# A-Kokolis/Hermes

Hardware: AMD Instinct MI355X
Metric: replicated KVS ops/s (reads+writes committed) (higher is better)
Workload: dtype u8

## Files before the change

### hermes_amd/csrc/hkv_batch.hip

```cpp
#include <hip/hip_runtime.h>

#include <algorithm>
#include <cstdio>
#include <cstdlib>
#include <cstring>

#include "hkv_batch_dev.h"

namespace hkv {

__host__ __device__ constexpr int rounds_for(int type, bool rmw)
{
    return type == kVals || (type == kLocal && !rmw) ? 0 : 2;
}

enum : uint8_t { kIvRaise = 1, kIvEq = 2, kIvWrite = 4, kIvCand = 8, kIvApply = 16 };
constexpr int64_t kInvDirectMax = 1 << 23;

enum : uint8_t { kAkMatch = 1 };

__device__ __forceinline__ uint8_t ack_opcode(uint8_t in) { return in == kLastAckSuccess ? in : kAckSuccess; }

__device__ __forceinline__ uint8_t inv_opcode(uint8_t in, bool oog)
{
// ... 1012 lines not shown
            const unsigned long long v = ((unsigned long long)(~a.rtag0) << 32) | (uint32_t)gi[k];
            const unsigned long long old = atomicExch(a.fw + fw_index(a, phys[k]), v);
            if ((uint32_t)(old >> 32) == ~a.rtag0 && a.error_flags) atomicOr(a.error_flags, 16u);
        }
        uint8_t *entry = a.log + phys[k];
        Ctx c = make_ctx(a);
        uint8_t idx = 0;
        if (TYPE == kAcks) {
            uint8_t *xx;
            elem_at(a, (uint32_t)gi[k], xx, idx, c);
        }
        Meta t = m[k];
        dispatch<SV>(TYPE, x, entry, idx, t, c);
        if (!meta_equal(t, m[k])) meta_store(entry, t);
    }
}

__device__ __forceinline__ uint4 load_chunk(const uint8_t *x, int q, int32_t esz)
{
    if (16 * q + 16 <= esz) return *reinterpret_cast<const uint4 *>(x + 16 * q);
    if (16 * q + 8 <= esz) {
        const uint64_t t = *reinterpret_cast<const uint64_t *>(x + 16 * q);
        return make_uint4((uint32_t)t, (uint32_t)(t >> 32), 0u, 0u);
    }
    return make_uint4(0u, 0u, 0u, 0u);
}

__device__ __forceinline__ bool chunk_equal(const uint4 &a, const uint4 &b)
{
    return a.x == b.x && a.y == b.y && a.z == b.z && a.w == b.w;
}

template <int TYPE, bool IL = false>
__global__ __launch_bounds__(64) void k_unique_lds(BatchArgs a)
{
    constexpr int P = 1;
    constexpr int E = 16 * P;
    __shared__ uint4 sops[E * 4];
    __shared__ uint4 sln[E * 4];
    __shared__ uint32_t sent[E];
    __shared__ uint8_t sprb[E];
    const int tid = threadIdx.x, q = tid & 3, gbase = tid & ~3;
    const int64_t i0 = (int64_t)blockIdx.x * E;
    const int64_t n_live = a.offsets ? (int64_t)a.offsets[a.n_batches] : a.n;
    uint64_t key[P];
    bool probe[P], ok[P], live[P];
    uint64_t phys[P];
    uint4 ln[P], op[P];
    int te[P];
#pragma unroll
    for (int k = 0; k < P; ++k) {
        te[k] = k * 16 + (tid >> 2);
        const int64_t i = i0 + te[k];
        live[k] = i < a.n && i < n_live;
        op[k] = live[k] ? load_chunk(a.elems + i * a.esz, q, a.esz) : make_uint4(0u, 0u, 0u, 0u);
        sops[te[k] * 4 + q] = op[k];
    }
#pragma unroll
    for (int k = 0; k < P; ++k) {
        key[k] = (uint64_t)(uint32_t)__shfl((int)op[k].x, 0, 4) | ((uint64_t)(uint32_t)__shfl((int)op[k].y, 0, 4) << 32);
        const uint32_t h0 = (uint32_t)__shfl((int)op[k].z, 0, 4);
        probe[k] = false;
        const int64_t i = i0 + te[k];
        if (live[k] && (a.offsets || in_count(a, (uint32_t)i))) {
            if (!skip_elem_os(TYPE, (uint8_t)h0, (uint8_t)(h0 >> 8))) {
                probe[k] = true;
            } else if (TYPE == kInvs && a.ns_idx && q == 0) {
                int64_t start;
                const int32_t b = batch_of(a, i, start);
                atomicMax(&a.ns_idx[b], (int32_t)(i - start));
            }
        }
    }
    uint8_t *home[P];
    lookup_pair<P, IL>(a, key, probe, q, gbase, ok, phys, ln, home);
#pragma unroll
    for (int k = 0; k < P; ++k) {
        Meta m;
        const uint64_t ek = line_key_meta(ln[k], m);
        const bool hit = ok[k] && ek == key[k];
        sln[te[k] * 4 + q] = ln[k];
        if (q == 0) {
            sent[te[k]] = hit ? (uint32_t)(phys[k] / a.g.entry_unit) : kNone;
            sprb[te[k]] = probe[k];
        }
    }
    __syncthreads();
    if (tid < E && i0 + tid < n_live) {
        const int64_t i = i0 + tid;
        uint8_t *x = reinterpret_cast<uint8_t *>(&sops[tid * 4]);
        uint8_t *ent = reinterpret_cast<uint8_t *>(&sln[tid * 4]);
        const uint32_t e = sent[tid];
        if (e != kNone) {
            if (a.check_unique) {
                const unsigned long long v = ((unsigned long long)(~a.rtag0) << 32) | (uint32_t)i;
                const unsigned long long old = atomicExch(a.fw + fw_index(a, phys_of(a, e)), v);
                if ((uint32_t)(old >> 32) == ~a.rtag0 && a.error_flags) atomicOr(a.error_flags, 16u);
            }
            Ctx c = make_ctx(a);
            int done = -1;
            if (TYPE == kAcks) c.rw_done = &done;
            Meta m;
            meta_load(ent, m);
            Meta t = m;
            dispatch<31>(TYPE, x, ent, 0, t, c);
            if (!meta_equal(t, m)) meta_store(ent, t);
            if (TYPE == kAcks && done >= 0 && a.rw) {
                uint8_t *xx;
                uint8_t idx;
                elem_at(a, (uint32_t)i, xx, idx, c);
                complete_rw_slot(c, done);
            }
        } else if (sprb[tid]) {
            x[9] = kMiss;
        }
    }
    __syncthreads();
#pragma unroll
    for (int k = 0; k < P; ++k) {
        if (!live[k]) continue;
        uint4 w = sops[te[k] * 4 + q];
        if (TYPE == kInvs && a.ack_out) {
            uint8_t *y = a.ack_out + (i0 + te[k]) * a.ack_out_size;
            const uint32_t hz = sops[te[k] * 4].z;
            const uint8_t oc = (uint8_t)hz;
            const bool full = oc == kOpInvAbort && a.ack_out_size >= (uint32_t)a.esz;
            if (oc == kInvSuccess || full) {
                uint4 c = w;
                if (q == 0)
                    c.z = (hz & ~0xFFFFu) | (oc == kInvSuccess ? kOpAck : kOpInvAbort) |
                          ((uint32_t)(uint8_t)a.g.machine_id << 8);
                if (q == 0 || (full && 16 * q < a.esz)) {
                    if (16 * q + 16 <= a.esz || q == 0) *reinterpret_cast<uint4 *>(y + 16 * q) = c;
                    else *reinterpret_cast<uint64_t *>(y + 16 * q) = (uint64_t)c.x | ((uint64_t)c.y << 32);
                }
            } else if (q == 0) {
                y[8] = kEmpty;
            }
            if (q == 0 && (oc == kInvSuccess || oc == kOpInvAbort || oc == kOpMembChange))
                w.z = (w.z & ~0xFFu) | kEmpty;
        }
        if (!chunk_equal(w, op[k])) {
            uint8_t *xg = a.elems + (i0 + te[k]) * a.esz + 16 * q;
            if (16 * q + 16 <= a.esz) *reinterpret_cast<uint4 *>(xg) = w;
            else *reinterpret_cast<uint64_t *>(xg) = (uint64_t)w.x | ((uint64_t)w.y << 32);
        }
        if (ok[k] && q > 0) {
            const uint4 l = sln[te[k] * 4 + q];
            if (!chunk_equal(l, ln[k])) reinterpret_cast<uint4 *>(IL ? home[k] : a.log + phys[k])[q] = l;
        }
    }
}

template <int TYPE, int RMAX, int CH, bool IL = false>
__global__ __launch_bounds__(64) void k_unique_rows(BatchArgs a)
{
    constexpr int P = kLookupPair;
    constexpr int E = 16 * P;
    __shared__ uint4 sops[RMAX][E * CH];
    __shared__ uint4 sln[E * 4];
    __shared__ uint32_t sent[E];
    __shared__ uint8_t spart[E];
    const int tid = threadIdx.x, q = tid & 3, gbase = tid & ~3;
    const int64_t i0 = (int64_t)blockIdx.x * E;
    const int R = a.n_rows < RMAX ? a.n_rows : RMAX;
    const int64_t n_live = a.offsets ? (int64_t)a.offsets[a.n_batches] : a.n;
    uint64_t key[P];
    bool probe[P], ok[P], live[P];
    uint64_t phys[P];
    uint4 ln[P], op[RMAX][P];
    uint32_t part[P];
    int te[P];
#pragma unroll
    for (int k = 0; k < P; ++k) {
        te[k] = k * 16 + (tid >> 2);
        const int64_t i = i0 + te[k];
        live[k] = i < a.n && i < n_live && (a.offsets || in_count(a, (uint32_t)i));
#pragma unroll
        for (int r = 0; r < RMAX; ++r) {
            const bool on = live[k] && r < R && r != a.skip_row;
            op[r][k] = on && q < CH ? load_chunk(a.elems + (r * a.row_stride + i) * a.esz, q, a.esz)
                                    : make_uint4(0u, 0u, 0u, 0u);
            if (q < CH) sops[r][te[k] * CH + q] = op[r][k];
        }
    }
#pragma unroll
    for (int k = 0; k < P; ++k) {
        uint64_t kk = 0;
        uint32_t p = 0;
        bool mismatch = false;
#pragma unroll
        for (int r = 0; r < RMAX; ++r) {
            const uint64_t kr = (uint64_t)(uint32_t)__shfl((int)op[r][k].x, 0, 4) |
                                ((uint64_t)(uint32_t)__shfl((int)op[r][k].y, 0, 4) << 32);
            const uint32_t h0 = (uint32_t)__shfl((int)op[r][k].z, 0, 4);
            if (!live[k] || r >= R || r == a.skip_row || (uint8_t)h0 == 0) continue;
            if (skip_elem_os(TYPE, (uint8_t)h0, (uint8_t)(h0 >> 8))) continue;
            if (p && kr != kk) mismatch = true;
            if (!p) kk = kr;
            p |= 1u << r;
        }
        if (mismatch && q == 0 && a.error_flags) atomicOr(a.error_flags, 16u);
        key[k] = kk;
        part[k] = mismatch ? 0u : p;
        probe[k] = part[k] != 0;
    }
    uint8_t *home[P];
    lookup_pair<P, IL>(a, key, probe, q, gbase, ok, phys, ln, home);
#pragma unroll
    for (int k = 0; k < P; ++k) {
        Meta m;
        const uint64_t ek = line_key_meta(ln[k], m);
        const bool hit = ok[k] && ek == key[k];
        sln[te[k] * 4 + q] = ln[k];
        if (q == 0) {
            sent[te[k]] = hit ? (uint32_t)(phys[k] / a.g.entry_unit) : kNone;
            spart[te[k]] = (uint8_t)part[k];
        }
    }
    __syncthreads();
    if (tid < E && i0 + tid < n_live) {
        const int64_t i = i0 + tid;
        uint8_t *ent = reinterpret_cast<uint8_t *>(&sln[tid * 4]);
        const uint32_t e = sent[tid];
        const uint32_t p = spart[tid];
        if (e != kNone && p) {
            if (a.check_unique) {
                const unsigned long long v = ((unsigned long long)(~a.rtag0) << 32) | (uint32_t)i;
                const unsigned long long old = atomicExch(a.fw + fw_index(a, phys_of(a, e)), v);
                if ((uint32_t)(old >> 32) == ~a.rtag0 && a.error_flags) atomicOr(a.error_flags, 16u);
            }
            Ctx c = make_ctx(a);
            int done = -1;
            if (TYPE == kAcks) c.rw_done = &done;
            Meta m;
            meta_load(ent, m);
            Meta t = m;
#pragma unroll
            for (int r = 0; r < RMAX; ++r)
                if ((p >> r) & 1u) dispatch<31>(TYPE, reinterpret_cast<uint8_t *>(&sops[r][tid * CH]), ent, 0, t, c);
            if (!meta_equal(t, m)) meta_store(ent, t);
            if (TYPE == kAcks && done >= 0 && a.rw) {
                uint8_t *xx;
                uint8_t idx;
                elem_at(a, (uint32_t)i, xx, idx, c);
                complete_rw_slot(c, done);
            }
        } else {
#pragma unroll
            for (int r = 0; r < RMAX; ++r)
                if ((p >> r) & 1u) reinterpret_cast<uint8_t *>(&sops[r][tid * CH])[9] = kMiss;
        }
    }
    __syncthreads();
#pragma unroll
    for (int k = 0; k < P; ++k) {
        if (!live[k]) continue;
#pragma unroll
        for (int r = 0; r < RMAX; ++r) {
            if (r >= R || r == a.skip_row || q >= CH) continue;
            uint4 w = sops[r][te[k] * CH + q];
            if (TYPE == kAcks && CH == 1 && a.ack_out) {
                const uint8_t oc = (uint8_t)w.z;
                uint4 v = make_uint4(0u, 0u, (uint32_t)kEmpty, 0u);
                if (oc != 0 && oc != kAckSuccess && oc != kOpMembChange && oc != kEmpty)
                    v = make_uint4(w.x, w.y, (w.z & ~0xFFFFu) | (uint32_t)kOpVal | ((uint32_t)(uint8_t)a.g.machine_id << 8), w.w);
                *reinterpret_cast<uint4 *>(a.ack_out + (r * a.row_stride + i0 + te[k]) * 16) = v;
                if (oc != 0 && oc != kEmpty) w.z = (w.z & ~0xFFu) | (uint32_t)kEmpty;
            }
            if (!chunk_equal(w, op[r][k])) {
                uint8_t *xg = a.elems + (r * a.row_stride + i0 + te[k]) * a.esz + 16 * q;
                if (16 * q + 16 <= a.esz) *reinterpret_cast<uint4 *>(xg) = w;
                else *reinterpret_cast<uint64_t *>(xg) = (uint64_t)w.x | ((uint64_t)w.y << 32);
            }
        }
        if (ok[k] && q > 0) {
            const uint4 l = sln[te[k] * 4 + q];
            if (!chunk_equal(l, ln[k])) reinterpret_cast<uint4 *>(IL ? home[k] : a.log + phys[k])[q] = l;
        }
    }
}

constexpr int kUbElems = 16;
constexpr int kUbChunks = 20;
template <int TYPE>
__global__ __launch_bounds__(64) void k_unique_big(BatchArgs a)
{
    __shared__ uint4 sx[kUbElems * kUbChunks];
    __shared__ uint4 se[kUbElems * kUbChunks];
    constexpr int kPerLane = (kUbChunks + 3) / 4;
    uint4 x0[kPerLane], e0[kPerLane];
    const int tid = threadIdx.x, q = tid & 3, el = tid >> 2, gbase = tid & ~3;
    const int64_t i = (int64_t)blockIdx.x * kUbElems + el;
    const bool live = i < a.n;
    const int nch = (a.esz + 15) / 16;
    uint8_t *xg = a.elems + i * a.esz;
#pragma unroll
    for (int u = 0; u < kPerLane; ++u) {
        const int c = q + 4 * u;
        const uint4 v = live && c < nch ? load_chunk(xg, c, a.esz) : make_uint4(0u, 0u, 0u, 0u);
        if (c < nch) sx[el * kUbChunks + c] = v;
        x0[u] = v;
    }
    const uint4 c0 = sx[el * kUbChunks];
    const uint64_t key = (uint64_t)c0.x | ((uint64_t)c0.y << 32);
    bool probe = false;
    if (live && (a.offsets || in_count(a, (uint32_t)i))) {
        if (!skip_elem_os(TYPE, (uint8_t)c0.z, (uint8_t)(c0.z >> 8))) {
            probe = true;
        } else if (TYPE == kInvs && a.ns_idx && q == 0) {
            int64_t start;
            const int32_t b = batch_of(a, i, start);
            atomicMax(&a.ns_idx[b], (int32_t)(i - start));
        }
    }
    bool ok;
    uint64_t phys;
    uint4 ln;
    lookup_pair<1>(a, &key, &probe, q, gbase, &ok, &phys, &ln);
    Meta m0;
    const uint64_t ek = line_key_meta(ln, m0);
    const bool hit = ok && ek == key;
#pragma unroll
    for (int u = 0; u < kPerLane; ++u) e0[u] = make_uint4(0u, 0u, 0u, 0u);
    if (hit) {
        const uint4 *eg = reinterpret_cast<const uint4 *>(a.log + phys);
#pragma unroll
        for (int u = 0; u < kPerLane; ++u) {
            const int c = q + 4 * u;
            if (c >= kUbChunks) continue;
            const uint4 v = c < 4 ? ln : eg[c];
            se[el * kUbChunks + c] = v;
            e0[u] = v;
        }
    }
    __syncthreads();
    if (q == 0 && live) {
        uint8_t *x = reinterpret_cast<uint8_t *>(&sx[el * kUbChunks]);
        uint8_t *ent = reinterpret_cast<uint8_t *>(&se[el * kUbChunks]);
        if (hit) {
            if (a.check_unique) {
                const unsigned long long v = ((unsigned long long)(~a.rtag0) << 32) | (uint32_t)i;
                const unsigned long long old = atomicExch(a.fw + fw_index(a, phys), v);
                if ((uint32_t)(old >> 32) == ~a.rtag0 && a.error_flags) atomicOr(a.error_flags, 16u);
            }
            Ctx c = make_ctx(a);
            int done = -1;
            if (TYPE == kAcks) c.rw_done = &done;
            Meta m;
            meta_load(ent, m);
            Meta t = m;
            dispatch<287>(TYPE, x, ent, 0, t, c);
            if (!meta_equal(t, m)) meta_store(ent, t);
            if (TYPE == kAcks && done >= 0 && a.rw) {
                uint8_t *xx;
                uint8_t idx;
                elem_at(a, (uint32_t)i, xx, idx, c);
                complete_rw_slot(c, done);
            }
        } else if (probe) {
            x[9] = kMiss;
        }
    }
    __syncthreads();
    if (live) {
        const uint32_t hz = sx[el * kUbChunks].z;
        const uint8_t oc = (uint8_t)hz;
        if (TYPE == kInvs && a.ack_out) {
            uint8_t *y = a.ack_out + i * a.ack_out_size;
            const bool full = oc == kOpInvAbort && a.ack_out_size >= (uint32_t)a.esz;
            if (oc == kInvSuccess || full) {
                for (int c = q; c < (full ? nch : 1); c += 4) {
                    uint4 w = sx[el * kUbChunks + c];
                    if (c == 0)
                        w.z = (hz & ~0xFFFFu) | (oc == kInvSuccess ? kOpAck : kOpInvAbort) |
                              ((uint32_t)(uint8_t)a.g.machine_id << 8);
                    if (16 * c + 16 <= a.esz || c == 0) *reinterpret_cast<uint4 *>(y + 16 * c) = w;
                    else *reinterpret_cast<uint64_t *>(y + 16 * c) = (uint64_t)w.x | ((uint64_t)w.y << 32);
                }
            } else if (q == 0) {
                y[8] = kEmpty;
            }
        }
#pragma unroll
        for (int u = 0; u < kPerLane; ++u) {
            const int c = q + 4 * u;
            if (c >= nch) continue;
            uint4 w = sx[el * kUbChunks + c];
            if (TYPE == kInvs && a.ack_out && c == 0 && (oc == kInvSuccess || oc == kOpInvAbort || oc == kOpMembChange))
                w.z = (w.z & ~0xFFu) | kEmpty;
            if (chunk_equal(w, x0[u])) continue;
            if (16 * c + 16 <= a.esz) *reinterpret_cast<uint4 *>(xg + 16 * c) = w;
            else *reinterpret_cast<uint64_t *>(xg + 16 * c) = (uint64_t)w.x | ((uint64_t)w.y << 32);
        }
    }
    if (hit) {
        uint4 *eg = reinterpret_cast<uint4 *>(a.log + phys);
#pragma unroll
        for (int u = 0; u < kPerLane; ++u) {
            const int c = q + 4 * u;
            if (c >= kUbChunks) continue;
            const uint4 w = se[el * kUbChunks + c];
            if (c > 0 && !chunk_equal(w, e0[u])) eg[c] = w;
        }
    }
}

template <int TYPE, int SV>
__global__ __launch_bounds__(256) void k_resolve(BatchArgs a, int r)
{
    extern __shared__ uint64_t sx[];
    const bool kStage = SV == 31 && a.esz <= 16;
    const int64_t i = (int64_t)blockIdx.x * 256 + threadIdx.x;
    bool left = false;
    VCopy vc{nullptr, nullptr};
    VCopy *vcp = SV != 31 && a.g.st_value <= 320 ? &vc : nullptr;
    const bool wave_shadow = SV != 31 && vcp;
    bool cand = false;
    uint32_t prev = 0;
    if (i < a.n && a.st[i] == kStPend) {
        const uint32_t e = a.ent[i];
        const uint32_t f = first_cand(*fw_of(a, e), a.rtag0 + (uint32_t)r);
        prev = a.pf[i];
        if (f == kNone || (uint32_t)i <= f) {
            uint8_t *xg = a.elems + i * a.esz;
            uint8_t *xl = reinterpret_cast<uint8_t *>(sx) + threadIdx.x * (uint32_t)a.esz;
            if (kStage) copy_elem(xl, xg, a.esz);
// ... 748 lines not shown
    BatchLaunch bl{};
    return carve(bl, 0, cap, entry_size);
}

void batch_carve(BatchLaunch &bl, uint8_t *base, int64_t cap, uint32_t entry_size)
{
    carve(bl, reinterpret_cast<uintptr_t>(base), cap, entry_size);
}

size_t batch_fw_words(uint64_t log_cap) { return (size_t)(log_cap >> 6); }

uint32_t batch_max_epoch() { return (1u << 29) - 1; }

static BatchPlan plan_batch(const BatchLaunch &bl)
{
    BatchPlan p{};
    const int64_t n = bl.n;
    if (n <= 0) return p;
    const int32_t type = bl.type;
    const uint32_t sv = bl.g.st_value;
    const bool rmw = bl.g.rmw_enabled != 0;
    const bool geo64 = sv == 31 && bl.g.entry_size == 64;
    const bool local_type = type == kLocal || type == kLocalAfterMemb;
    p.sv = sv == 31 ? 31 : sv == 287 ? 287 : 0;
    p.big = bl.esz > 64;
    p.mixed = bl.hdr != nullptr;
    p.il = bl.line != nullptr;
    p.inv_direct = type == kInvs && !rmw && n < kInvDirectMax;
    p.ack_direct = type == kAcks && !rmw && n < (int64_t)kNone;
    p.ack_out = bl.ack_out && (type == kInvs || (type == kAcks && bl.n_rows > 0));
    p.state_out = local_type;
    p.opc = type == kLocal;
    p.fk = type == kLocal && rmw && p.big;
    p.rw_mirrors = type == kAcks;

    if ((bl.path == kPathSmall || (bl.path == kPathAuto && n <= kSmallMaxElems)) && n <= kSmallMaxElems) {
        p.engine = Engine::kSmall;
    } else if (type == kLocal && !rmw && bl.esz == 56 && geo64 && !bl.offsets) {
        p.engine = Engine::kLocalDirect;
        p.inline_instance = true;
    } else if (bl.n_rows > 0 && bl.unique) {
        p.engine = Engine::kRows;
        p.rmax = bl.n_rows <= 2 ? 2 : 8;
        p.ch = type == kInvs ? 4 : bl.esz <= 16 ? 1 : 4;
        p.inline_instance = geo64 && !local_type && bl.n_rows <= 8;
    } else if (bl.unique && (type == kInvs || type == kAcks)) {
        if (geo64 && bl.esz <= 64) {
            p.engine = Engine::kUniqueLds64;
            p.inline_instance = true;
        } else if (type == kInvs && sv == 287 && bl.g.entry_size == 320 && bl.esz <= 320) {
            p.engine = Engine::kUniqueLdsBig;
        } else {
            p.engine = Engine::kUniqueInPlace;
            if (p.ack_out) p.refuse = -1;
        }
    } else if (type == kVals) {
        p.engine = Engine::kValsOnePass;
        p.inline_instance = geo64;
    } else {
        p.lookup_head = local_type && n > kLookupHead ? kLookupHead : n;
        p.slab_threads = p.big ? 128 : 256;
        p.engine = p.ack_direct ? Engine::kRoundsAckDirect
                   : p.inv_direct ? Engine::kRoundsInvDirect
                   : p.big && type != kInvs ? Engine::kRoundsInPlace
                                            : Engine::kRoundsSlab;
    }
    if (p.il && !p.inline_instance) p.refuse = -1;
    if (bl.region_bytes && p.engine != Engine::kSmall) p.refuse = -1;
    p.node_suspected = p.engine != Engine::kSmall && type == kInvs && bl.ns_idx && bl.node_suspected;

    const uint32_t vend = (uint32_t)kOpValueOff + sv;
    if (!bl.patch) p.patches = Patches::kNone;
    else if (p.engine == Engine::kSmall) p.patches = Patches::kApplyFirst;
    else if (p.engine == Engine::kLocalDirect) p.patches = Patches::kByEngine;
    else if (type == kLocal && p.big && !bl.offsets && sv != 31 && sv <= kPirMaxValue && bl.esz % 8 == 0 &&
             (uint32_t)bl.esz >= vend && (uint32_t)bl.esz <= vend + 8)
        p.patches = Patches::kInResolve;
    else p.patches = Patches::kApplyFirst;
    return p;
}

bool batch_inline_capable(const BatchLaunch &bl) { return plan_batch(bl).inline_instance; }

static BatchArgs make_args(const BatchLaunch &bl, const BatchPlan &p)
{
#ifdef HKV_DEBUG_MODES
    static const int dbg_env = getenv("HKV_DBG") ? atoi(getenv("HKV_DBG")) : 0;
#else
    constexpr int dbg_env = 0;
#endif
    static const int check_unique_env = getenv("HKV_CHECK_UNIQUE") ? atoi(getenv("HKV_CHECK_UNIQUE")) : 0;
    BatchArgs a{};
    a.elems = bl.elems;
    a.counts = bl.counts;
    a.offsets = bl.offsets;
    a.index = bl.index;
    a.log = bl.log;
    a.rw = bl.rw;
    a.ns_idx = bl.ns_idx;
    a.fw = bl.fw;
    a.fx = bl.fx;
    a.fy = bl.fy;
    a.ft = bl.ft;
    a.fw_mask = (uint32_t)((bl.g.log_cap >> 6) - 1);
    a.ent = bl.ent;
    a.st = bl.st;
    a.pf = bl.pf;
    a.shadow = bl.shadow;
    a.mem = bl.mem;
    a.fbl = bl.fbl;
    a.ctr = bl.ctr;
    a.error_flags = bl.error_flags;
    a.g = bl.g;
    a.n = bl.n;
    a.rw_stride = bl.rw_stride;
    a.stride = bl.stride;
    a.esz = bl.esz;
    a.type = bl.type;
    a.rtag0 = bl.epoch << 3;
    a.ltag = (uint8_t)(bl.epoch % 255u + 1u);
    a.rounds = rounds_for(bl.type, bl.g.rmw_enabled != 0);
    a.inv_direct = p.inv_direct;
    a.ack_direct = p.ack_direct;
    a.g_membership = bl.g_membership;
    a.w_ack_init = bl.w_ack_init;
    a.node_suspected = bl.node_suspected;
    a.n_batches = bl.n_batches;
    a.host_src = bl.host_src;
    a.host_dst = bl.host_dst;
    a.dev_region = bl.dev_region;
    a.region_bytes = bl.region_bytes;
    a.done_flag = bl.done_flag;
    a.done_value = bl.done_value;
    a.hdr = bl.hdr;
    a.state_out = p.state_out ? bl.state_out : nullptr;
    a.opc = p.opc ? bl.opcode_in : nullptr;
    a.patch = p.patches == Patches::kInResolve || p.patches == Patches::kByEngine ? bl.patch : nullptr;
    a.fk = p.fk ? bl.fk : nullptr;
    a.hx = p.patches == Patches::kInResolve ? bl.hx : nullptr;
    a.rws = p.rw_mirrors ? bl.rw_state : nullptr;
    a.rwo = p.rw_mirrors ? bl.opcode_in : nullptr;
    a.n_rows = bl.n_rows;
    a.skip_row = bl.skip_row;
    a.row_stride = bl.row_stride;
    a.dbg = dbg_env;
    a.check_unique = check_unique_env;
    a.ack_out = p.ack_out ? bl.ack_out : nullptr;
    a.ack_out_size = bl.ack_out_size;
    a.line = bl.line;
    return a;
}

constexpr int kRowsElems = 16 * kLookupPair;
template <int T, int CH>
static void launch_rows(const BatchArgs &a, const BatchPlan &p, hipStream_t s)
{
    const unsigned lgrid = (unsigned)((a.n + kRowsElems - 1) / kRowsElems);
    with_bool(p.il, [&](auto il) {
        constexpr bool IL = decltype(il)::value;
        if (p.rmax == 2) hipLaunchKernelGGL((k_unique_rows<T, 2, CH, IL>), dim3(lgrid), dim3(64), 0, s, a);
        else hipLaunchKernelGGL((k_unique_rows<T, 8, CH, IL>), dim3(lgrid), dim3(64), 0, s, a);
    });
}

template <int T>
static void launch_unique_t(const BatchArgs &a, const BatchPlan &p, hipStream_t s)
{
    if (p.engine == Engine::kUniqueLds64) {
        const unsigned g1 = (unsigned)((a.n + 15) / 16);
        with_bool(p.il, [&](auto il) {
            hipLaunchKernelGGL((k_unique_lds<T, decltype(il)::value>), dim3(g1), dim3(64), 0, s, a);
        });
    } else {
        const unsigned ugrid1 = (unsigned)((a.n + 63) / 64);
        with_sv(p.sv, [&](auto v) {
            hipLaunchKernelGGL((k_unique<T, decltype(v)::value>), dim3(ugrid1), dim3(256), 0, s, a);
        });
    }
}

static int launch_unique(const BatchArgs &a, const BatchPlan &p, hipStream_t s)
{
    if (p.engine == Engine::kRows) {
        if (a.type == kInvs) launch_rows<kInvs, 4>(a, p, s);
        else if (p.ch == 1) launch_rows<kAcks, 1>(a, p, s);
        else launch_rows<kAcks, 4>(a, p, s);
    } else if (p.engine == Engine::kUniqueLdsBig) {
        hipLaunchKernelGGL(k_unique_big<kInvs>, dim3((unsigned)((a.n + kUbElems - 1) / kUbElems)), dim3(64), 0, s, a);
    } else if (a.type == kInvs) {
        launch_unique_t<kInvs>(a, p, s);
    } else {
        launch_unique_t<kAcks>(a, p, s);
    }
    return hipGetLastError() == hipSuccess ? 0 : -3;
}

template <int T, int V>
static int launch_rounds_tv(const BatchArgs &a, const BatchPlan &p, hipStream_t s)
{
    const unsigned grid = (unsigned)((a.n + 255) / 256);
    const unsigned cgrid = (unsigned)((a.n + 256 * kCandPer - 1) / (256 * kCandPer));
    const unsigned rgrid = (unsigned)((a.n + p.slab_threads - 1) / p.slab_threads);
    const size_t rlds = (size_t)p.slab_threads * (size_t)a.esz;
    if (p.big && rlds > 64 * 1024 &&
        hipFuncSetAttribute((const void *)k_resolve0<T, V, 128>, hipFuncAttributeMaxDynamicSharedMemorySize, (int)rlds) !=
            hipSuccess)
        return -3;
    if (p.engine == Engine::kRoundsInPlace) hipLaunchKernelGGL((k_resolve0_direct<T, V>), dim3(grid), dim3(256), 0, s, a);
    else if (p.big) hipLaunchKernelGGL((k_resolve0<T, V, 128>), dim3(rgrid), dim3(128), rlds, s, a);
    else hipLaunchKernelGGL((k_resolve0<T, V, 256>), dim3(rgrid), dim3(256), rlds, s, a);
    for (int r = 1; r <= a.rounds; ++r) {
        hipLaunchKernelGGL((k_cand<T>), dim3(cgrid), dim3(256), 0, s, a, r);
        hipLaunchKernelGGL((k_resolve<T, V>), dim3(grid), dim3(256), V == 31 ? 256 * a.esz : 0, s, a, r);
    }
    hipLaunchKernelGGL((k_commit<V>), dim3(grid), dim3(256), 0, s, a);
    if (a.rounds > 0) hipLaunchKernelGGL((k_fb_exec<T, V>), dim3(256), dim3(kFbThreads), 0, s, a);
    return 0;
}

template <int T>
static int launch_rounds_t(const BatchArgs &a, const BatchPlan &p, hipStream_t s)
{
    int rc = 0;
    with_sv(p.sv, [&](auto v) { rc = launch_rounds_tv<T, decltype(v)::value>(a, p, s); });
    return rc;
}

static int launch_rounds(const BatchArgs &a, const BatchPlan &p, hipStream_t s)
{
    const int64_t n = a.n;
    const unsigned grid = (unsigned)((n + 255) / 256);
    if (p.engine == Engine::kValsOnePass) {
        with_bool(p.il, [&](auto il) {
            hipLaunchKernelGGL(k_lookup<decltype(il)::value>, dim3((unsigned)((n + 63) / 64)), dim3(256), 0, s, a,
                               (int64_t)0, n);
        });
        return hipGetLastError() == hipSuccess ? 0 : -3;
    }
    const int64_t head = p.lookup_head;
    hipLaunchKernelGGL(k_lookup<>, dim3((unsigned)((head + 63) / 64)), dim3(256), 0, s, a, (int64_t)0, head);
    if (n > head) hipLaunchKernelGGL(k_lookup<>, dim3((unsigned)((n - head + 63) / 64)), dim3(256), 0, s, a, head, n);
    int rc = 0;
    if (p.engine == Engine::kRoundsAckDirect) {
        hipLaunchKernelGGL(k_ack_resolve, dim3(grid), dim3(256), 0, s, a);
    } else if (p.engine == Engine::kRoundsInvDirect) {
        hipLaunchKernelGGL(k_inv_resolve, dim3(grid), dim3(256), 0, s, a, (int64_t)0, n);
        with_sv(p.sv, [&](auto v) { hipLaunchKernelGGL((k_inv_commit<decltype(v)::value>), dim3(grid), dim3(256), 0, s, a); });
    } else {
        switch (a.type) {
        case kLocal: rc = launch_rounds_t<kLocal>(a, p, s); break;
        case kLocalAfterMemb: rc = launch_rounds_t<kLocalAfterMemb>(a, p, s); break;
        case kInvs: rc = launch_rounds_t<kInvs>(a, p, s); break;
        case kAcks: rc = launch_rounds_t<kAcks>(a, p, s); break;
        default: rc = launch_rounds_t<kVals>(a, p, s); break;
        }
    }
    if (rc) return rc;
    return hipGetLastError() == hipSuccess ? 0 : -3;
}

int launch_batch(BatchLaunch &bl, hipStream_t s)
{
    if (bl.n <= 0) return 0;
    const BatchPlan p = plan_batch(bl);
    if (p.refuse) return p.refuse;
    const BatchArgs a = make_args(bl, p);
    if (p.patches == Patches::kApplyFirst)
        hipLaunchKernelGGL(k_apply_patch, dim3((unsigned)((bl.n + 255) / 256)), dim3(256), 0, s, bl.elems, bl.patch, bl.n,
                           bl.esz, bl.g.st_value);
    int rc;
    switch (p.engine) {
    case Engine::kSmall: rc = launch_small(a, p, s); break;
    case Engine::kLocalDirect: rc = launch_local(a, p, s); break;
    case Engine::kRows:
    case Engine::kUniqueLds64:
    case Engine::kUniqueLdsBig:
    case Engine::kUniqueInPlace: rc = launch_unique(a, p, s); break;
    default: rc = launch_rounds(a, p, s); break;
    }
    if (rc) return rc;
    if (p.node_suspected) {
        hipLaunchKernelGGL(k_node_suspected, dim3((bl.n_batches + 255) / 256), dim3(256), 0, s, bl.elems, bl.ns_idx,
                           bl.node_suspected, bl.n_batches, bl.stride, bl.esz, bl.offsets);
        if (hipGetLastError() != hipSuccess) return -4;
    }
    return 0;
}

}
```

### hermes_amd/csrc/hkv_batch_dev.h

```cpp
#pragma once
#include <hip/hip_runtime.h>

#include <type_traits>

#include "hkv_exec.h"
#include "hkv_internal.h"
#include "hkv_table_dev.h"

namespace hkv {

constexpr uint32_t kNone = 0xFFFFFFFFu;
enum : uint8_t { kStDone = 0, kStCommit = 1, kStPend = 2, kStDefer = 3 };
enum { kCtrFbM = 1, kCtrFbL = 2, kCtrDefer = 3 };

struct BatchArgs {
    uint8_t *elems;
    const int32_t *counts;
    const int32_t *offsets;
    const uint8_t *index;
    uint8_t *log;
    uint8_t *rw;
    int32_t *ns_idx;
    unsigned long long *fw;
    unsigned long long *fx, *fy;
// ... 17 lines not shown
    uint8_t ltag;
    int32_t rounds;
    int32_t inv_direct;
    int32_t ack_direct;
    uint8_t g_membership;
    uint8_t w_ack_init;
    int32_t *node_suspected;
    int32_t n_batches;
    const uint8_t *host_src;
    uint8_t *host_dst;
    uint8_t *dev_region;
    uint64_t region_bytes;
    uint32_t *done_flag;
    uint32_t done_value;
    unsigned long long *prof;
    const SmallBatch *hdr;
    uint8_t *state_out;
    const uint8_t *opc;
    const uint8_t *patch;
    uint16_t *fk;
    uint64_t *hx;
    uint8_t *rws;
    const uint8_t *rwo;
    int32_t n_rows, skip_row;
    int64_t row_stride;
    int32_t dbg;
    int32_t check_unique;
    uint8_t *ack_out;
    uint32_t ack_out_size;
    uint8_t *line;
};

enum class Engine : uint8_t {
    kSmall,
    kLocalDirect,
    kRows,
    kUniqueLds64,
    kUniqueLdsBig,
    kUniqueInPlace,
    kValsOnePass,
    kRoundsAckDirect,
    kRoundsInvDirect,
    kRoundsSlab,
    kRoundsInPlace,
};
enum class Patches : uint8_t {
    kNone,
    kApplyFirst,
    kByEngine,
    kInResolve,
};
constexpr uint32_t kPirMaxValue = 320;
constexpr uint32_t kWaveWordsMaxValue = 8 * 62;
static_assert(kPirMaxValue <= kWaveWordsMaxValue, "wave_value_copies_n ignores VCopy::fill: handle it there first");
struct BatchPlan {
    int refuse;
    Engine engine;
    Patches patches;
    int sv;
    int rmax, ch;
    int slab_threads;
    int64_t lookup_head;
    bool big;
    bool mixed;
    bool inv_direct, ack_direct;
    bool ack_out;
    bool state_out, opc;
    bool fk;
    bool rw_mirrors;
    bool node_suspected;
    bool il;
    bool inline_instance;
};

int launch_small(const BatchArgs &a, const BatchPlan &p, hipStream_t s);
int launch_local(const BatchArgs &a, const BatchPlan &p, hipStream_t s);

template <class F>
inline void with_sv(int sv, F &&f)
{
    if (sv == 31) f(std::integral_constant<int, 31>{});
    else if (sv == 287) f(std::integral_constant<int, 287>{});
    else f(std::integral_constant<int, 0>{});
}
template <class F>
inline void with_bool(bool b, F &&f)
{
    if (b) f(std::true_type{});
    else f(std::false_type{});
}

__device__ __forceinline__ Ctx make_ctx(const BatchArgs &a)
{
    Ctx c;
    c.g = a.g;
    c.g_membership = a.g_membership;
    c.w_ack_init = a.w_ack_init;
    c.rw = nullptr;
    c.rws = nullptr;
    c.rw_done = nullptr;
    c.vc = nullptr;
    return c;
}

__device__ __forceinline__ uint64_t phys_of(const BatchArgs &a, uint32_t e) { return (uint64_t)e * a.g.entry_unit; }
__device__ __forceinline__ uint8_t *entry_of(const BatchArgs &a, uint32_t e) { return a.log + phys_of(a, e); }

struct __attribute__((aligned(8))) U64x2 {
    uint64_t a, b;
};

template <int TYPE>
__device__ __forceinline__ uint8_t absorbing_state()
{
    return TYPE == kVals ? kValid : kWrite;
}

template <int TYPE>
__device__ __forceinline__ Meta after_first(const BatchArgs &a, const Meta &m0, uint32_t f, int f_is_put)
{
    Meta m1 = m0;
    m_set_state(m1, absorbing_state<TYPE>());
    if (TYPE != kLocal || a.g.skew == 0) return m1;
    uint8_t foc = f_is_put ? (uint8_t)kOpPut : a.elems[(int64_t)f * a.esz + 8];
    if (a.hx && !f_is_put) {
        const uint64_t pb = *reinterpret_cast<const uint64_t *>(a.patch + (int64_t)f * 16 + 8);
        if ((pb >> 48) & 0xFFu) foc = (uint8_t)pb;
    }
    if (foc != kOpGet) {
        m1.ver += 2;
        m_set_cid(m1, (uint8_t)a.g.machine_id);
    } else {
        m_set_state(m1, kReplay);
    }
    return m1;
}

__device__ __forceinline__ int32_t batch_of(const BatchArgs &a, int64_t i, int64_t &start)
{
    if (!a.offsets) {
        const int32_t b = (int32_t)(i / a.stride);
        start = (int64_t)b * a.stride;
        return b;
    }
    int lo = 0, hi = a.n_batches - 1;
    while (lo < hi) {
        const int mid = (lo + hi + 1) >> 1;
        if (a.offsets[mid] <= i) lo = mid; else hi = mid - 1;
    }
    start = a.offsets[lo];
    return lo;
}

__device__ __forceinline__ void elem_at(const BatchArgs &a, uint32_t i, uint8_t *&x, uint8_t &idx, Ctx &c)
{
    c.rw = nullptr;
    c.rws = nullptr;
    idx = 0;
    if (a.rw || !a.offsets) {
        int64_t start;
        const int32_t b = batch_of(a, i, start);
        idx = (uint8_t)(i - start);
        c.rw = a.rw ? a.rw + (int64_t)b * a.rw_stride : nullptr;
        c.rws = a.rws ? a.rws + (int64_t)b * (a.rw_stride / a.g.op_size) : nullptr;
        c.rwo = a.rwo ? a.rwo + (int64_t)b * (a.rw_stride / a.g.op_size) : nullptr;
    }
    x = a.elems + (int64_t)i * a.esz;
}

__device__ __forceinline__ void note_state(const BatchArgs &a, int64_t i, const uint8_t *x)
{
    if (a.state_out) a.state_out[i] = x[9];
}

__device__ __forceinline__ uint32_t fw_index(const BatchArgs &a, uint64_t phys)
{
    return (uint32_t)(((phys >> 6) * 0x9E3779B1ull) & a.fw_mask);
}
__device__ __forceinline__ unsigned long long *fw_of(const BatchArgs &a, uint32_t e) { return a.fw + fw_index(a, phys_of(a, e)); }

__device__ __forceinline__ uint32_t first_cand(unsigned long long f, uint32_t rtag)
{
    return (uint32_t)(f >> 32) == ~rtag ? (uint32_t)f : kNone;
}

__device__ __forceinline__ void offer(unsigned long long *f, uint32_t rtag, uint32_t i)
{
    const unsigned long long v = ((unsigned long long)(~rtag) << 32) | i;
    if (v < __hip_atomic_load(f, __ATOMIC_RELAXED, __HIP_MEMORY_SCOPE_AGENT)) atomicMin(f, v);
}

__device__ __forceinline__ uint8_t *shadow_of(const BatchArgs &a, uint32_t i)
{
    return a.shadow + (size_t)i * a.g.entry_size;
}

__device__ __forceinline__ void copy_entry(uint8_t *dst, const uint8_t *src, uint32_t bytes)
{
    struct __attribute__((aligned(8))) W16 {
        uint64_t a, b;
    };
    uint32_t o = 0;
    for (; o + 16 <= bytes; o += 16) *reinterpret_cast<W16 *>(dst + o) = *reinterpret_cast<const W16 *>(src + o);
    if (o < bytes) *reinterpret_cast<uint64_t *>(dst + o) = *reinterpret_cast<const uint64_t *>(src + o);
}

template <int TYPE, int SV>
__device__ __forceinline__ void apply_to_shadow(const BatchArgs &a, uint8_t *x, uint32_t i, const uint8_t *src)
{
    uint8_t *sh = shadow_of(a, i);
    Meta m;
    meta_load(src, m);
    if (SV == 31) {
        const uint4 *s4 = reinterpret_cast<const uint4 *>(src);
        uint4 *d4 = reinterpret_cast<uint4 *>(sh);
        const uint4 w0 = s4[0], w1 = s4[1], w2 = s4[2], w3 = s4[3];
        d4[0] = w0;
        d4[1] = w1;
        d4[2] = w2;
        d4[3] = w3;
    } else {
        copy_entry(sh, src, a.g.entry_size);
    }
    Ctx c = make_ctx(a);
    uint8_t *xg;
    uint8_t idx;
    elem_at(a, i, xg, idx, c);
    if (x) dispatch<SV>(TYPE, x, sh, idx, m, c);
    else dispatch<SV>(TYPE, xg, sh, idx, m, c);
    meta_store(sh, m);
}

__device__ __forceinline__ bool patch_valid(uint64_t pb) { return ((pb >> 48) & 0xFFu) != 0; }

__device__ __forceinline__ bool in_count(const BatchArgs &a, uint32_t i)
{
    if (!a.counts) return true;
    const uint32_t b = i / (uint32_t)a.stride;
    return (int32_t)(i - b * (uint32_t)a.stride) < a.counts[b];
}

__device__ __forceinline__ uint64_t line_key_meta(const uint4 &ln, Meta &m)
{
    const uint64_t ek = (uint64_t)(uint32_t)__shfl((int)ln.z, 0, 4) | ((uint64_t)(uint32_t)__shfl((int)ln.w, 0, 4) << 32);
    m.w4 = (uint32_t)__shfl((int)ln.x, 1, 4);
    m.w5 = (uint32_t)__shfl((int)ln.y, 1, 4);
    m.ver = (uint32_t)__shfl((int)ln.z, 1, 4);
    const uint32_t w7 = (uint32_t)__shfl((int)ln.w, 1, 4);
    const uint32_t b32 = (uint32_t)__shfl((int)ln.x, 2, 4) & 0xFFu;
    m.llw_cid = (uint8_t)w7;
    m.llw_ver = (w7 >> 8) | (b32 << 24);
    return ek;
}

constexpr int kLookupPair = 2;
template <int P = kLookupPair, bool IL = false, bool F = false>
__device__ __forceinline__ void lookup_core(const BatchArgs &a, const uint64_t *key, const bool *probe, int q,
                                            int gbase, bool *ok, uint64_t *phys, uint4 *ln, unsigned long long *fwv,
                                            uint8_t **home, bool *inl)
{
    uint4 v[P], ev[P];
#pragma unroll
    for (int k = 0; k < P; ++k) {
        if (IL) {
            const uint4 *l = line_words(a.line, bucket_of(a.g, key[k]));
            v[k] = probe[k] ? l[q] : make_uint4(0u, 0u, 0u, 0u);
            ev[k] = probe[k] ? l[4 + q] : make_uint4(0u, 0u, 0u, 0u);
        } else {
            v[k] = probe[k] ? bucket_words(a.index, bucket_of(a.g, key[k]))[q] : make_uint4(0u, 0u, 0u, 0u);
        }
    }
    bool il[P];
#pragma unroll
    for (int k = 0; k < P; ++k) {
        const uint64_t s0 = u64_of(v[k].x, v[k].y), s1 = u64_of(v[k].z, v[k].w);
        const uint32_t tag = key_tag(key[k]);
        const bool mt0 = probe[k] && (s0 & 1u) && ((uint32_t)(s0 >> 1) & 0x7FFFFFu) == tag;
        const bool mt1 = probe[k] && (s1 & 1u) && ((uint32_t)(s1 >> 1) & 0x7FFFFFu) == tag;
        const uint32_t g0 = (uint32_t)(__ballot(mt0) >> gbase) & 0xFu;
        const uint32_t g1 = (uint32_t)(__ballot(mt1) >> gbase) & 0xFu;
        uint32_t o = 0;
#pragma unroll
        for (int l = 0; l < 4; ++l) o |= ((g0 >> l) & 1u) << (2 * l) | ((g1 >> l) & 1u) << (2 * l + 1);
        const int first = o ? __ffs(o) - 1 : 0;
        const uint64_t raw = group_slot_word(slot_off_raw(s0), slot_off_raw(s1), first), off = off_of<IL>(raw);
        ok[k] = probe[k] && o && in_log_window(a.g, off);
        phys[k] = off & a.g.log_mask;
        il[k] = off_is_inline<IL>(raw) && ok[k];
    }
#pragma unroll
    for (int k = 0; k < P; ++k) {
        if (IL) {
            ln[k] = ev[k];
            if (!il[k]) ln[k] = ok[k] ? reinterpret_cast<const uint4 *>(a.log + phys[k])[q] : make_uint4(0u, 0u, 0u, 0u);
            if (home) home[k] = il[k] ? line_entry(a.line, a.g, key[k]) : a.log + phys[k];
            if (inl) inl[k] = il[k];
        } else {
            ln[k] = ok[k] ? reinterpret_cast<const uint4 *>(a.log + phys[k])[q] : make_uint4(0u, 0u, 0u, 0u);
            if (home) home[k] = a.log + phys[k];
            if (inl) inl[k] = false;
        }
        if (F) fwv[k] = ok[k] && q == 0 ? a.fw[fw_index(a, phys[k])] : ~0ull;
    }
}

template <int P = kLookupPair, bool IL = false>
__device__ __forceinline__ void lookup_pair(const BatchArgs &a, const uint64_t *key, const bool *probe, int q,
                                            int gbase, bool *ok, uint64_t *phys, uint4 *ln, uint8_t **home = nullptr,
                                            bool *inl = nullptr)
{
    lookup_core<P, IL, false>(a, key, probe, q, gbase, ok, phys, ln, nullptr, home, inl);
}

template <int P, bool IL = false>
__device__ __forceinline__ void lookup_pair_f(const BatchArgs &a, const uint64_t *key, const bool *probe, int q,
                                              int gbase, bool *ok, uint64_t *phys, uint4 *ln, unsigned long long *fwv,
                                              uint8_t **home = nullptr, bool *inl = nullptr)
{
    lookup_core<P, IL, true>(a, key, probe, q, gbase, ok, phys, ln, fwv, home, inl);
}

}
```

Measured before the change: 5.003 billion.

## Add wide ack rows kernel with flat loads and cooperative batch locate

Adds a wider variant of the unique-rows kernel (64 elements per block, one lane per element) for the ack path with single-chunk ops and two rows, used only when the batch is large. Op headers are loaded flat per lane and read back from shared memory instead of through 4-lane shuffles. For acks with read-write slots, the owning batch is found once per block by a cooperative 64-way search over batch offsets, interleaved with the index lookup loads, which replaces the per-element binary search in elem_at. This adds code complexity, extra offset loads and a barrier, and the new path only runs above a size threshold.

Result: faster. 5.083 billion, median of 6 (+1.6%).

```diff
diff --git a/hermes_amd/csrc/hkv_batch.hip b/hermes_amd/csrc/hkv_batch.hip
--- a/hermes_amd/csrc/hkv_batch.hip
+++ b/hermes_amd/csrc/hkv_batch.hip
@@ -1188,10 +1188,9 @@
     }
 }
 
-template <int TYPE, int RMAX, int CH, bool IL = false>
+template <int TYPE, int RMAX, int CH, int P = kLookupPair, bool IL = false>
 __global__ __launch_bounds__(64) void k_unique_rows(BatchArgs a)
 {
-    constexpr int P = kLookupPair;
     constexpr int E = 16 * P;
     __shared__ uint4 sops[RMAX][E * CH];
     __shared__ uint4 sln[E * 4];
@@ -1201,23 +1200,58 @@
     const int64_t i0 = (int64_t)blockIdx.x * E;
     const int R = a.n_rows < RMAX ? a.n_rows : RMAX;
     const int64_t n_live = a.offsets ? (int64_t)a.offsets[a.n_batches] : a.n;
+    const auto is_live = [&](int64_t i) { return i < a.n && i < n_live && (a.offsets || in_count(a, (uint32_t)i)); };
     uint64_t key[P];
     bool probe[P], ok[P], live[P];
     uint64_t phys[P];
-    uint4 ln[P], op[RMAX][P];
+    constexpr bool FLAT = P == 4 && CH == 1;
+    const bool flat_live = FLAT && is_live(i0 + tid);
+    uint4 ln[P], op[RMAX][FLAT ? 1 : P];
     uint32_t part[P];
     int te[P];
 #pragma unroll
     for (int k = 0; k < P; ++k) {
         te[k] = k * 16 + (tid >> 2);
-        const int64_t i = i0 + te[k];
-        live[k] = i < a.n && i < n_live && (a.offsets || in_count(a, (uint32_t)i));
+        live[k] = is_live(i0 + te[k]);
+    }
+    if (FLAT) {
 #pragma unroll
         for (int r = 0; r < RMAX; ++r) {
-            const bool on = live[k] && r < R && r != a.skip_row;
-            op[r][k] = on && q < CH ? load_chunk(a.elems + (r * a.row_stride + i) * a.esz, q, a.esz)
-                                    : make_uint4(0u, 0u, 0u, 0u);
-            if (q < CH) sops[r][te[k] * CH + q] = op[r][k];
+            const bool on = flat_live && r < R && r != a.skip_row;
+            op[r][0] = on ? load_chunk(a.elems + (r * a.row_stride + i0 + tid) * a.esz, 0, a.esz) : make_uint4(0u, 0u, 0u, 0u);
+        }
+    } else {
+#pragma unroll
+        for (int k = 0; k < (FLAT ? 1 : P); ++k) {
+            const int64_t i = i0 + te[k];
+#pragma unroll
+            for (int r = 0; r < RMAX; ++r) {
+                const bool on = live[k] && r < R && r != a.skip_row;
+                op[r][k] = on && q < CH ? load_chunk(a.elems + (r * a.row_stride + i) * a.esz, q, a.esz)
+                                        : make_uint4(0u, 0u, 0u, 0u);
+            }
+        }
+    }
+    const bool locate = TYPE == kAcks && a.offsets && a.rw;
+    int32_t blo = 0, bhi = a.n_batches - 1, bsample = 0;
+    const auto sample = [&]() {
+        const int32_t s = kary_sample(blo, bhi, tid);
+        const int32_t v = a.offsets[s < bhi ? s : bhi];
+        return s <= bhi ? v : INT32_MAX;
+    };
+    const auto narrow = [&]() { kary_narrow(blo, bhi, __popcll(__ballot((int64_t)bsample <= i0))); };
+    const bool step1 = locate && bhi - blo >= kRowsWindow / 2;
+    if (step1) bsample = sample();
+    if (FLAT) {
+#pragma unroll
+        for (int r = 0; r < RMAX; ++r) sops[r][tid] = op[r][0];
+        __syncthreads();
+    } else {
+#pragma unroll
+        for (int k = 0; k < (FLAT ? 1 : P); ++k) {
+#pragma unroll
+            for (int r = 0; r < RMAX; ++r)
+                if (q < CH) sops[r][te[k] * CH + q] = op[r][k];
         }
     }
 #pragma unroll
@@ -1227,9 +1261,17 @@
         bool mismatch = false;
 #pragma unroll
         for (int r = 0; r < RMAX; ++r) {
-            const uint64_t kr = (uint64_t)(uint32_t)__shfl((int)op[r][k].x, 0, 4) |
-                                ((uint64_t)(uint32_t)__shfl((int)op[r][k].y, 0, 4) << 32);
-            const uint32_t h0 = (uint32_t)__shfl((int)op[r][k].z, 0, 4);
+            uint64_t kr;
+            uint32_t h0;
+            if (FLAT) {
+                const uint4 h = sops[r][te[k]];
+                kr = (uint64_t)h.x | ((uint64_t)h.y << 32);
+                h0 = h.z;
+            } else {
+                const uint4 &h = op[r][FLAT ? 0 : k];
+                kr = (uint64_t)(uint32_t)__shfl((int)h.x, 0, 4) | ((uint64_t)(uint32_t)__shfl((int)h.y, 0, 4) << 32);
+                h0 = (uint32_t)__shfl((int)h.z, 0, 4);
+            }
             if (!live[k] || r >= R || r == a.skip_row || (uint8_t)h0 == 0) continue;
             if (skip_elem_os(TYPE, (uint8_t)h0, (uint8_t)(h0 >> 8))) continue;
             if (p && kr != kk) mismatch = true;
@@ -1242,7 +1284,22 @@
         probe[k] = part[k] != 0;
     }
     uint8_t *home[P];
-    lookup_pair<P, IL>(a, key, probe, q, gbase, ok, phys, ln, home);
+    bool step2 = false;
+    lookup_pair_beside<P, IL>(a, key, probe, q, gbase, ok, phys, ln, home, [&]() {
+        if (step1) narrow();
+        step2 = locate && bhi - blo >= kRowsWindow / 2;
+        if (step2) bsample = sample();
+    });
+    if (step2) narrow();
+    while (locate && bhi - blo >= kRowsWindow / 2) {
+        bsample = sample();
+        narrow();
+    }
+    int32_t w0 = INT32_MAX, w1 = INT32_MAX;
+    if (locate) {
+        if (blo + tid < a.n_batches) w0 = a.offsets[blo + tid];
+        if (blo + 64 + tid < a.n_batches) w1 = a.offsets[blo + 64 + tid];
+    }
 #pragma unroll
     for (int k = 0; k < P; ++k) {
         Meta m;
@@ -1253,6 +1310,13 @@
             sent[te[k]] = hit ? (uint32_t)(phys[k] / a.g.entry_unit) : kNone;
             spart[te[k]] = (uint8_t)part[k];
         }
+    }
+    int32_t pb = -1;
+    if (locate) {
+        const int32_t k0 = __popcll(__ballot((int64_t)w0 <= i0)) - 1;
+        const auto win = [&](int32_t j) { return __builtin_amdgcn_readlane(j < 64 ? w0 : w1, j & 63); };
+        int32_t b;
+        if (rows_window_batch(win, blo, k0 > 0 ? k0 : 0, i0 + tid, i0 + E - 1, b)) pb = b;
     }
     __syncthreads();
     if (tid < E && i0 + tid < n_live) {
@@ -1277,9 +1341,13 @@
                 if ((p >> r) & 1u) dispatch<31>(TYPE, reinterpret_cast<uint8_t *>(&sops[r][tid * CH]), ent, 0, t, c);
             if (!meta_equal(t, m)) meta_store(ent, t);
             if (TYPE == kAcks && done >= 0 && a.rw) {
-                uint8_t *xx;
-                uint8_t idx;
-                elem_at(a, (uint32_t)i, xx, idx, c);
+                if (pb >= 0) {
+                    batch_rw(a, pb, c);
+                } else {
+                    uint8_t *xx;
+                    uint8_t idx;
+                    elem_at(a, (uint32_t)i, xx, idx, c);
+                }
                 complete_rw_slot(c, done);
             }
         } else {
@@ -1289,26 +1357,34 @@
         }
     }
     __syncthreads();
+    const auto put_back = [&](int r, int pos, int c, const uint4 &was) {
+        uint4 w = sops[r][pos * CH + c];
+        if (TYPE == kAcks && CH == 1 && a.ack_out) {
+            const uint8_t oc = (uint8_t)w.z;
+            uint4 v = make_uint4(0u, 0u, (uint32_t)kEmpty, 0u);
+            if (oc != 0 && oc != kAckSuccess && oc != kOpMembChange && oc != kEmpty)
+                v = make_uint4(w.x, w.y, (w.z & ~0xFFFFu) | (uint32_t)kOpVal | ((uint32_t)(uint8_t)a.g.machine_id << 8), w.w);
+            *reinterpret_cast<uint4 *>(a.ack_out + (r * a.row_stride + i0 + pos) * 16) = v;
+            if (oc != 0 && oc != kEmpty) w.z = (w.z & ~0xFFu) | (uint32_t)kEmpty;
+        }
+        if (!chunk_equal(w, was)) {
+            uint8_t *xg = a.elems + (r * a.row_stride + i0 + pos) * a.esz + 16 * c;
+            if (16 * c + 16 <= a.esz) *reinterpret_cast<uint4 *>(xg) = w;
+            else *reinterpret_cast<uint64_t *>(xg) = (uint64_t)w.x | ((uint64_t)w.y << 32);
+        }
+    };
+    if (FLAT && flat_live) {
+#pragma unroll
+        for (int r = 0; r < RMAX; ++r)
+            if (r < R && r != a.skip_row) put_back(r, tid, 0, op[r][0]);
+    }
 #pragma unroll
     for (int k = 0; k < P; ++k) {
         if (!live[k]) continue;
 #pragma unroll
         for (int r = 0; r < RMAX; ++r) {
-            if (r >= R || r == a.skip_row || q >= CH) continue;
-            uint4 w = sops[r][te[k] * CH + q];
-            if (TYPE == kAcks && CH == 1 && a.ack_out) {
-                const uint8_t oc = (uint8_t)w.z;
-                uint4 v = make_uint4(0u, 0u, (uint32_t)kEmpty, 0u);
-                if (oc != 0 && oc != kAckSuccess && oc != kOpMembChange && oc != kEmpty)
-                    v = make_uint4(w.x, w.y, (w.z & ~0xFFFFu) | (uint32_t)kOpVal | ((uint32_t)(uint8_t)a.g.machine_id << 8), w.w);
-                *reinterpret_cast<uint4 *>(a.ack_out + (r * a.row_stride + i0 + te[k]) * 16) = v;
-                if (oc != 0 && oc != kEmpty) w.z = (w.z & ~0xFFu) | (uint32_t)kEmpty;
-            }
-            if (!chunk_equal(w, op[r][k])) {
-                uint8_t *xg = a.elems + (r * a.row_stride + i0 + te[k]) * a.esz + 16 * q;
-                if (16 * q + 16 <= a.esz) *reinterpret_cast<uint4 *>(xg) = w;
-                else *reinterpret_cast<uint64_t *>(xg) = (uint64_t)w.x | ((uint64_t)w.y << 32);
-            }
+            if (FLAT || r >= R || r == a.skip_row || q >= CH) continue;
+            put_back(r, te[k], q, op[r][FLAT ? 0 : k]);
         }
         if (ok[k] && q > 0) {
             const uint4 l = sln[te[k] * 4 + q];
@@ -2363,14 +2439,26 @@
 }
 
 constexpr int kRowsElems = 16 * kLookupPair;
+constexpr int kRowsWideElems = 16 * 4;
+constexpr int64_t kRowsWidePositions = (int64_t)28 * 256 * kRowsElems + 1;
 template <int T, int CH>
 static void launch_rows(const BatchArgs &a, const BatchPlan &p, hipStream_t s)
 {
     const unsigned lgrid = (unsigned)((a.n + kRowsElems - 1) / kRowsElems);
     with_bool(p.il, [&](auto il) {
         constexpr bool IL = decltype(il)::value;
-        if (p.rmax == 2) hipLaunchKernelGGL((k_unique_rows<T, 2, CH, IL>), dim3(lgrid), dim3(64), 0, s, a);
-        else hipLaunchKernelGGL((k_unique_rows<T, 8, CH, IL>), dim3(lgrid), dim3(64), 0, s, a);
+        if constexpr (T == kAcks && CH == 1) {
+            if (p.rmax == 2 && a.n >= kRowsWidePositions) {
+                const unsigned wgrid = (unsigned)((a.n + kRowsWideElems - 1) / kRowsWideElems);
+                hipLaunchKernelGGL((k_unique_rows<T, 2, CH, 4, IL>), dim3(wgrid), dim3(64), 0, s, a);
+                return;
+            }
+        }
+        if (p.rmax == 2) {
+            hipLaunchKernelGGL((k_unique_rows<T, 2, CH, kLookupPair, IL>), dim3(lgrid), dim3(64), 0, s, a);
+        } else {
+            hipLaunchKernelGGL((k_unique_rows<T, 8, CH, kLookupPair, IL>), dim3(lgrid), dim3(64), 0, s, a);
+        }
     });
 }
 
diff --git a/hermes_amd/csrc/hkv_batch_dev.h b/hermes_amd/csrc/hkv_batch_dev.h
--- a/hermes_amd/csrc/hkv_batch_dev.h
+++ b/hermes_amd/csrc/hkv_batch_dev.h
@@ -193,6 +193,43 @@
     return lo;
 }
 
+constexpr int kRowsWindow = 128;
+__host__ __device__ inline int32_t kary_stride(int32_t lo, int32_t hi) { return (hi - lo + 63) >> 6; }
+__host__ __device__ inline int32_t kary_sample(int32_t lo, int32_t hi, int s) { return lo + (s + 1) * kary_stride(lo, hi); }
+__host__ __device__ inline void kary_narrow(int32_t &lo, int32_t &hi, int32_t c)
+{
+    const int32_t step = kary_stride(lo, hi);
+    lo += c * step;
+    if (lo + step - 1 < hi) hi = lo + step - 1;
+}
+template <class Count>
+__host__ __device__ inline int32_t kary_last_le(int32_t n, int32_t span, Count &&count)
+{
+    int32_t lo = 0, hi = n - 1;
+    while (hi - lo > span) kary_narrow(lo, hi, count(lo, hi));
+    return lo;
+}
+
+template <class Win>
+__host__ __device__ inline bool rows_window_batch(Win &&win, int32_t lo, int32_t k0, int64_t i, int64_t i_max, int32_t &b)
+{
+    int32_t k = k0;
+    for (int32_t j = k0 + 1; j < kRowsWindow; ++j) {
+        const int32_t v = win(j);
+        if ((int64_t)v > i_max) break;
+        if ((int64_t)v <= i) k = j;
+    }
+    b = lo + k;
+    return k + 1 < kRowsWindow;
+}
+
+__device__ __forceinline__ void batch_rw(const BatchArgs &a, int32_t b, Ctx &c)
+{
+    c.rw = a.rw ? a.rw + (int64_t)b * a.rw_stride : nullptr;
+    c.rws = a.rws ? a.rws + (int64_t)b * (a.rw_stride / a.g.op_size) : nullptr;
+    c.rwo = a.rwo ? a.rwo + (int64_t)b * (a.rw_stride / a.g.op_size) : nullptr;
+}
+
 __device__ __forceinline__ void elem_at(const BatchArgs &a, uint32_t i, uint8_t *&x, uint8_t &idx, Ctx &c)
 {
     c.rw = nullptr;
@@ -202,9 +239,7 @@
         int64_t start;
         const int32_t b = batch_of(a, i, start);
         idx = (uint8_t)(i - start);
-        c.rw = a.rw ? a.rw + (int64_t)b * a.rw_stride : nullptr;
-        c.rws = a.rws ? a.rws + (int64_t)b * (a.rw_stride / a.g.op_size) : nullptr;
-        c.rwo = a.rwo ? a.rwo + (int64_t)b * (a.rw_stride / a.g.op_size) : nullptr;
+        batch_rw(a, b, c);
     }
     x = a.elems + (int64_t)i * a.esz;
 }
@@ -295,10 +330,13 @@
 }
 
 constexpr int kLookupPair = 2;
-template <int P = kLookupPair, bool IL = false, bool F = false>
+struct NothingBeside {
+    __device__ __forceinline__ void operator()() const {}
+};
+template <int P = kLookupPair, bool IL = false, bool F = false, class Beside = NothingBeside>
 __device__ __forceinline__ void lookup_core(const BatchArgs &a, const uint64_t *key, const bool *probe, int q,
                                             int gbase, bool *ok, uint64_t *phys, uint4 *ln, unsigned long long *fwv,
-                                            uint8_t **home, bool *inl)
+                                            uint8_t **home, bool *inl, Beside &&beside = Beside{})
 {
     uint4 v[P], ev[P];
 #pragma unroll
@@ -311,6 +349,7 @@
             v[k] = probe[k] ? bucket_words(a.index, bucket_of(a.g, key[k]))[q] : make_uint4(0u, 0u, 0u, 0u);
         }
     }
+    beside();
     bool il[P];
 #pragma unroll
     for (int k = 0; k < P; ++k) {
@@ -353,6 +392,14 @@
     lookup_core<P, IL, false>(a, key, probe, q, gbase, ok, phys, ln, nullptr, home, inl);
 }
 
+template <int P, bool IL, class Beside>
+__device__ __forceinline__ void lookup_pair_beside(const BatchArgs &a, const uint64_t *key, const bool *probe, int q,
+                                                   int gbase, bool *ok, uint64_t *phys, uint4 *ln, uint8_t **home,
+                                                   Beside &&beside)
+{
+    lookup_core<P, IL, false>(a, key, probe, q, gbase, ok, phys, ln, nullptr, home, nullptr, beside);
+}
+
 template <int P, bool IL = false>
 __device__ __forceinline__ void lookup_pair_f(const BatchArgs &a, const uint64_t *key, const bool *probe, int q,
                                               int gbase, bool *ok, uint64_t *phys, uint4 *ln, unsigned long long *fwv,
```
